# kemingy/rabitq

Measured on AMD Instinct MI355X. Metric: queries/sec at recall@10>=0.95, 100Mx128; HBM GB/s on popcount scan, higher is better.
Workload: dtype exact integer dot (fp6 MFMA, v_dot8_u32_u4) + f32

## Files before the change

### rabitq_amd/csrc/common.h

```cpp
#pragma once
#include <hip/hip_runtime.h>
#include <stdint.h>

#pragma clang fp contract(off)

#define RQ_WAVE 64

typedef float f32x2 __attribute__((ext_vector_type(2)));

__host__ __device__ __forceinline__ int32_t ord32_from_f32(float x) {
    int32_t bits = __builtin_bit_cast(int32_t, x);
    uint32_t mask = ((uint32_t)(bits >> 31)) >> 1;
    return bits ^ (int32_t)mask;
}
__host__ __device__ __forceinline__ float ord32_to_f32(int32_t key) {
    uint32_t mask = ((uint32_t)(key >> 31)) >> 1;
    return __builtin_bit_cast(float, key ^ (int32_t)mask);
}
__host__ __device__ __forceinline__ uint32_t ord32_biased(float x) {
    return (uint32_t)ord32_from_f32(x) ^ 0x80000000u;
}
__host__ __device__ __forceinline__ float ord32_unbias(uint32_t u) {
    return ord32_to_f32((int32_t)(u ^ 0x80000000u));
}

__device__ __forceinline__ float reduce8_lanes(float acc) {
    acc = acc + __shfl_xor(acc, 4, 8);
    acc = acc + __shfl_xor(acc, 1, 8);
    acc = acc + __shfl_xor(acc, 2, 8);
    return acc;
}
__device__ __forceinline__ float reduce8_regs(const float (&a)[8]) {
    float c0 = a[0] + a[4], c1 = a[1] + a[5], c2 = a[2] + a[6], c3 = a[3] + a[7];
    return (c0 + c1) + (c2 + c3);
}

__device__ __forceinline__ int32_t cvtps_epi32(float x) {
    if (x >= -2147483648.0f && x < 2147483648.0f) return (int32_t)rintf(x);
    return (int32_t)0x80000000;
}

struct __attribute__((aligned(16))) SurvRec {
    uint32_t pos;
    uint32_t slot;
    float rough;
    float accurate;
};
__device__ __forceinline__ uint64_t surv_key(const SurvRec &r) {
    return ((uint64_t)r.slot << 32) | r.pos;
}

struct __attribute__((aligned(16))) RunRec {
    uint32_t pos;
    uint32_t slot;
// ... 192 lines not shown
```

### rabitq_amd/csrc/host_plan.h

```cpp
#pragma once
struct QueryParams {
    uint32_t nq, len, probe, topk;
    bool heuristic;
    uint32_t cap, hcap;
    const float *thr_init = nullptr;
    bool seg_final = false;
    bool ext_lists = false;
    const rq_filter *filter = nullptr;
    bool range = false;
};

struct QueryIO {
    const float *d_q = nullptr;
    float *out_dist = nullptr;
    uint32_t *out_id = nullptr, *out_n = nullptr;
    const uint32_t *ext_cluster = nullptr;
    const float *ext_dist = nullptr;
    const float *thr_init = nullptr;
};
struct QueryCall {
    rq_index *idx = nullptr;
    const rq_filter *filter = nullptr;
    uint32_t len = 0, probe = 0, topk = 0;
    bool heuristic = false;
// ... 23 lines not shown
#define RQ_MAX_PROBE 16384u
#define RQ_SB_FILT_REACH 65536u

#define RQ_PREP_SHAPES(X) X(128, 16, 2, 16, 2) X(64, 16, 1, 16, 4) X(256, 32, 2, 8, 2) X(512, 32, 4, 8, 1) X(768, 32, 6, 8, 1) X(1024, 32, 8, 8, 1)

struct StagePlan {
    uint32_t s_lo, s_hi;
    uint64_t span, est_pairs;
    bool matrix;
    bool cluster_major;
    bool ranked;
    bool additive;
    bool arena_stage;
    bool placed;
    bool want_table;
    uint32_t slot_hi, stage_pairs;
    uint32_t dense_cells;
    uint32_t tile, tiles_per_group;
};

struct PassPlan {
    uint32_t nprobe, npairs;
    uint32_t dbg;
    bool large;
    bool small;
    uint32_t sb_nstages, sb_lo[RQ_SB_MAX_STAGES], sb_hi[RQ_SB_MAX_STAGES], sb_final_lo;
    bool sb_whole, sb_fill_final;
    bool will_list;
    bool placed;
    bool fin_additive;
// ... 10 lines not shown
    const uint64_t total_max = std::min<uint64_t>((uint64_t)nprobe * idx->max_list_len, idx->n);
    uint64_t lo = 0, hi = first_hi;
    const uint64_t avg = std::max<uint64_t>(1, idx->n / std::max<uint32_t>(idx->nonempty_lists, 1));
    uint64_t settle = std::min(settle_cap, std::max<uint64_t>(avg, std::min<uint64_t>(idx->max_list_len, 16 * avg)));
    if (pl.large) settle = std::max<uint64_t>(1, settle * settle_pct / 100);
    while (lo < total_max) {
        const bool last = hi >= total_max || lo >= settle || pl.nstages + 1 == RQ_MAX_STAGES;
        pl.st[pl.nstages++] = StagePlan{(uint32_t)lo, last ? 0xFFFFFFFFu : (uint32_t)hi};
        if (last) break;
        lo = hi;
        hi = std::min<uint64_t>(hi * growth, 0xFFFFFFF0ull);
        if (lo < 2 * avg && 2 * hi > 2 * avg) hi = 2 * avg;
        if (lo < settle && hi > settle) hi = settle;
    }
}

static void plan_pass(const rq_index *idx, const QueryParams &qp, bool has_row_map, bool ext_lists, PassPlan &pl) {
    const uint32_t dim = idx->dim, k = idx->k, W = idx->W;
    const uint32_t nq = qp.nq, nprobe = std::min(qp.probe, k), topk = qp.topk;
    const uint32_t npairs = nq * nprobe;
    const rq_filter *filt = qp.filter;
    const bool large = rq_large_batch(nq), fused = scan_is_fused(W);
    pl = PassPlan{};
    pl.nprobe = nprobe, pl.npairs = npairs, pl.large = large;
    const uint32_t min_len = filt ? 0u : idx->min_list_len;
    const int impl = g_scan_impl.load();
    pl.dbg = (uint32_t)g_scan_dbg.load();
    const int gate_opt = g_scan_gate.load(), rank_opt = g_group_rank.load(), tt_opt = g_scan_tile_table.load(), gopt = g_stage_growth.load();
    const bool dense_opt = g_dense_dir.load() != 0, additive_loose = idx->additive_loose.load() != 0;
    const uint64_t settle_pct = (uint64_t)g_stage_settle_pct.load();
// ... 48 lines not shown
                     (gate_opt == 2 || !additive_loose);
        s.slot_hi = nprobe;
        if (s.cluster_major && min_len > 0 && !ext_lists && s.s_hi != 0xFFFFFFFFu)
            s.slot_hi = (uint32_t)std::min<uint64_t>(nprobe, (uint64_t)(s.s_hi - 1) / min_len + 1);
        s.stage_pairs = nq * s.slot_hi;
        s.ranked = s.cluster_major && k <= 32768 &&
                   (rank_opt == 2 || (rank_opt == 1 && s.stage_pairs >= 16 * RQ_RANK_ITEMS && s.stage_pairs / RQ_RANK_ITEMS >= k / 256));
        s.tile = s.matrix ? scan_mfma_tile(W, s.arena_stage, s.additive) : scan_tile(W);
        s.tiles_per_group = ceil_div(std::min<uint64_t>(idx->max_list_len, s.s_hi), s.tile);
        const uint64_t grid_blocks = (uint64_t)k * s.tiles_per_group, real_tiles = idx->n / s.tile + k;
        s.want_table = s.cluster_major && fused && s.s_hi >= idx->max_list_len && (tt_opt == 2 || (tt_opt == 1 && grid_blocks > 4 * real_tiles));
        if (large && !s.matrix && fused && dense_opt && s.s_hi != 0xFFFFFFFFu && !(qp.seg_final && s.span > qp.cap)) {
            const uint64_t cells = (uint64_t)((s.s_hi - 1) >> 6) - (s.s_lo >> 6) + 2ull * s.slot_hi + 2;
            if (cells <= qp.cap) s.dense_cells = (uint32_t)cells;
        }
    }

#define RQ_X(D, LP, R, PPB, PP) \
    if (dim == D) pl.prep_lp = LP, pl.prep_r = R, pl.prep_ppb = PPB, pl.prep_pp = PP;
    RQ_PREP_SHAPES(RQ_X)
#undef RQ_X
    const bool prep_dim = pl.prep_lp != 0;
    pl.will_list = !pl.small && (filt || (idx->nonempty_lists * 2 < k && npairs >= 65536)) && g_pair_split.load() != 0 && prep_dim;
    if (g_prep_placement.load() != 0 && !pl.small && !filt && !ext_lists && !has_row_map && !qp.thr_init && !qp.seg_final && !pl.will_list &&
        prep_dim && fused && pl.nstages) {
        StagePlan &fin = pl.st[pl.nstages - 1];
        pl.placed = fin.s_hi == 0xFFFFFFFFu && fin.matrix && fin.ranked;
        for (uint32_t i = 0; i + 1 < pl.nstages; ++i) pl.placed = pl.placed && !pl.st[i].matrix;
        fin.placed = pl.placed;
        pl.fin_additive = pl.placed && fin.additive;
// ... 13 lines not shown

    if (pl.dbg & 16384) {
        fprintf(stderr, "[rabitq_hip] plan: pass nq=%u nprobe=%u large=%d small=%d will_list=%d placed=%d fin_additive=%d qn_slots=%u nstages=%u seg_final=%d sb_nstages=%u sb_whole=%d\n",
                nq, nprobe, (int)pl.large, (int)pl.small, (int)pl.will_list, (int)pl.placed, (int)pl.fin_additive, pl.qn_slots, pl.nstages, (int)qp.seg_final,
                pl.small ? pl.sb_nstages : 0u, (int)(pl.small && pl.sb_whole));
        for (uint32_t i = 0; pl.small && i < pl.sb_nstages; ++i)
            fprintf(stderr, "[rabitq_hip] plan: sb_stage=%u lo=%u hi=%u\n", i, pl.sb_lo[i], pl.sb_hi[i]);
        for (uint32_t i = 0; i < pl.nstages; ++i) {
            const StagePlan &s = pl.st[i];
            fprintf(stderr, "[rabitq_hip] stage %u: [%u, %u) span %llu est_pairs %llu %s\n", i, s.s_lo, s.s_hi, (unsigned long long)s.span,
                    (unsigned long long)s.est_pairs, s.matrix ? "matrix cores" : (s.cluster_major ? "VALU, list-major" : "VALU, pair-major"));
            if (s.placed) fprintf(stderr, "[rabitq_hip] stage %u: placed ahead of the quantisation (%s gate)\n", i, pl.fin_additive ? "additive" : "bf16");
            fprintf(stderr, "[rabitq_hip] plan: stage=%u lo=%u hi=%u matrix=%d cluster_major=%d ranked=%d additive=%d arena=%d placed=%d table=%d dense_cells=%u slot_hi=%u\n",
                    i, s.s_lo, s.s_hi, (int)s.matrix, (int)s.cluster_major, (int)s.ranked, (int)s.additive, (int)s.arena_stage, (int)s.placed, (int)s.want_table,
                    s.dense_cells, s.slot_hi);
        }
    }
}
```

### rabitq_amd/csrc/host_query.h

```cpp
#pragma once
static rq_status ws_prepare(const rq_index *idx, Workspace &ws, const QueryParams &qp) {
    const uint32_t nprobe = std::min(qp.probe, idx->k);
    const uint64_t nq = qp.nq, npairs = nq * nprobe;
    RQC(ws_ensure_stream(ws));
    RQC(ws.qpad.ensure(nq * idx->dim));
    RQC(ws.y.ensure(nq * idx->dim));
    if (!qp.ext_lists) RQC(ws.dist.ensure(nq * idx->k));
    RQC(ws.probe_dist.ensure(npairs));
    RQC(ws.probe_cluster.ensure(npairs));
    RQC(ws.scal.ensure(npairs));
    if (!scan_is_fused(idx->W)) RQC(ws.planes.ensure(npairs * 4 * idx->W));
    RQC(ws.qnib.ensure(npairs * 8 * idx->W));
    RQC(ws.qf6.ensure(npairs * 12 * idx->W));
    RQC(ws.rough_cnt.ensure(nq));
    RQC(ws.totals.ensure(16));
    RQC(ws.stat.ensure(256));
    RQC(ws.recs.ensure((npairs + 32ull * idx->k + 32) * (12ull * idx->W + 2 + RQ_REC_TAIL)));
    RQC(ws.grp_cnt.ensure(idx->k + 4));
    RQC(ws.grp_start.ensure(idx->k + 1));
    RQC(ws.q_hist.ensure(idx->k + 2));
    RQC(ws.q_start.ensure(idx->k + 2));
    RQC(ws.q_order.ensure(nq));
    RQC(ws.thr.ensure(nq));
    RQC(ws.surv.ensure(nq * qp.cap));
// ... 496 lines not shown
                flags |= 2u;
            }
            auto finish = topk < 64 ? sb_finish_kernel<true> : sb_finish_kernel<false>;
            finish<<<nq, fin_threads, (size_t)dim * sizeof(float) + (2 * RQ_SBF_RUNS + RQ_SBF_RECS) * 16, st>>>(
                ws.surv.p, ws.runs.p, ws.surv_cnt.p, seg, idx->view(), qpad, dim, topk, rs, probe_cluster, nprobe, flags,
                idx->map_ids.p, io.out_dist, io.out_id, io.out_n, ws.rough_cnt.p, ws.totals.p);
            sb_results_done = true;
        } else {
            auto finish = qp.heuristic ? stage_finish_kernel<true> : stage_finish_kernel<false>;
            finish<<<nq, fin_threads, (size_t)dim * sizeof(float), st>>>(ws.surv.p, ws.runs.p, ws.surv_cnt.p, seg, idx->view(), qpad, dim, topk, rs,
                                                                         probe_cluster, nprobe, flags);
        }
        pf.end();
    }

    void stage_finish_large(StageRun &r) {
        const uint32_t dense_cells = r.s.dense_cells;
        const QSeg &seg = r.seg;
        pf.begin(PF_RERANK);
        const uint32_t gx = std::max(1u, std::min(16u, 4096u / std::max(nq, 1u)));
        const bool prefilter = (r.no > 0 || qp.thr_init) && !(pl.dbg & 512);
        if (idx->base_q8.p && prefilter)
            accurate_filtered8_kernel<<<dim3(gx, nq), 256, (size_t)dim * sizeof(float) + (nprobe <= RQ_ACC8_LDS_PROBES ? (size_t)nprobe * 16 : 0), st>>>(
                ws.surv.p, ws.surv_cnt.p, seg, idx->base.p, idx->base_q8.p, idx->list_q8.p, qpad, dim, rerank_order, ws.thr.p,
                probe_cluster, nprobe, ws.nshadow.p, k);
        else if (idx->base_h.p && prefilter)
            accurate_filtered_kernel<<<dim3(gx, nq), 256, (size_t)dim * sizeof(float), st>>>(
                ws.surv.p, ws.surv_cnt.p, seg, idx->base.p, idx->base_h.p, qpad, dim, rerank_order, ws.thr.p,
                ws.nshadow.p);
        else if (idx->split_rows && prefilter)
            accurate_split_kernel<<<dim3(gx, nq), 256, (size_t)dim * sizeof(float) + (nprobe <= RQ_ACC8_LDS_PROBES ? (size_t)nprobe * 16 : 0), st>>>(
                ws.surv.p, ws.surv_cnt.p, seg, idx->view(), qpad, dim, rerank_order, ws.thr.p, probe_cluster, nprobe, ws.nshadow.p);
        else
            accurate_kernel<<<dim3(gx, nq), 256, (size_t)dim * sizeof(float), st>>>(ws.surv.p, ws.surv_cnt.p, seg, idx->view(), qpad, dim,
                                                                                    rerank_order, probe_cluster, nprobe);
        if (qp.range)
            range_count_kernel<<<ceil_div(nq, 4), 256, 0, st>>>(ws.surv.p, ws.surv_cnt.p, qp.cap, ws.thr.p, nq, ws.range_hits.p, ws.need.p,
// ... 68 lines not shown
    const size_t total_span = pf.spans.size() ? pf.spans.size() - 1 : 0;
    if (pl.small) {
        RQC(c.small_front());
    } else {
        RQC(c.rotate_coarse());
        if (pl.placed) RQC(c.place_final());
        pf.begin(PF_PREP);
        RQC(c.quantise());
        RQC(c.orders_state());
        pf.end();
    }
    for (uint32_t i = 0; i < pl.nstages; ++i) {
        StageRun r{pl.st[i], i};
        RQC(c.stage_group_fill(r));
        RQC(c.stage_scan(r));
        if (!qp.range && !pl.large && qp.cap <= 4 * RQ_DEFAULT_CAP) c.stage_finish_small(r);
        else c.stage_finish_large(r);
    }
    RQC(c.results(total_span));
    if (defer) return RQ_OK;
    return finish_pass(idx, ws, res, prof_acc);
}
```

### rabitq_amd/csrc/host_state.h

```cpp
#pragma once
static thread_local std::string g_err;
static rq_status fail(rq_status s, const std::string &msg) {
    g_err = msg;
    return s;
}
#define HIPC(expr)                                                                                   \
    do {                                                                                             \
        hipError_t _e = (expr);                                                                      \
        if (_e != hipSuccess)                                                                        \
            return fail(_e == hipErrorOutOfMemory ? RQ_ERR_OOM : RQ_ERR_HIP,                         \
                        std::string(#expr) + ": " + hipGetErrorString(_e));                          \
    } while (0)
#define RQC(expr)                        \
    do {                                 \
        rq_status _s = (expr);           \
        if (_s != RQ_OK) return _s;      \
    } while (0)

static rq_status ensure_device() {
    int count = 0;
    hipError_t e = hipGetDeviceCount(&count);
    if (e != hipSuccess || count == 0)
        return fail(RQ_ERR_NO_DEVICE, "no HIP device visible (librabitq_hip has no CPU fallback)");
    return RQ_OK;
// ... 699 lines not shown
    static hipError_t err = hipSuccess;
    static const char *what = "";
    std::call_once(once, [] {
        auto set = [&](const void *fn, int bytes, const char *name) {
            if (err != hipSuccess) return;
            err = hipFuncSetAttribute(fn, hipFuncAttributeMaxDynamicSharedMemorySize, bytes);
            if (err != hipSuccess) what = name;
        };
        set(reinterpret_cast<const void *>(select_probe_kernel), 140 * 1024, "select_probe_kernel");
        set(reinterpret_cast<const void *>(coarse_dist_kernel<4>), 140 * 1024, "coarse_dist_kernel<4>");
        set(reinterpret_cast<const void *>(coarse_dist_kernel<8>), 140 * 1024, "coarse_dist_kernel<8>");
        set(reinterpret_cast<const void *>(assign_generic_kernel<8>), 140 * 1024, "assign_generic_kernel<8>");
        set(reinterpret_cast<const void *>(merge_smallest_u64_kernel), 16384 * 8, "merge_smallest_u64_kernel");
        set(reinterpret_cast<const void *>(group_rank_kernel), 32768 * 4, "group_rank_kernel");
        set(reinterpret_cast<const void *>(sb_front_kernel), 140 * 1024, "sb_front_kernel");
        set(reinterpret_cast<const void *>(sort_runs_mid_kernel), RQ_SORT_MID_LDS_WORDS * 8, "sort_runs_mid_kernel");
        set(reinterpret_cast<const void *>(range_sort_block_kernel<1024, RQ_RANGE_TILE>), RQ_RANGE_TILE * 8, "range_sort_block_kernel");
        set(reinterpret_cast<const void *>(range_sort_tile_kernel), RQ_RANGE_TILE * 8, "range_sort_tile_kernel");
        set(reinterpret_cast<const void *>(assign_approx_kernel<6, 1>), (int)assign_lds_bytes<6, 1>(), "assign_approx_kernel<6,1>");
        set(reinterpret_cast<const void *>(assign_approx_kernel<8, 1>), (int)assign_lds_bytes<8, 1>(), "assign_approx_kernel<8,1>");
        set(reinterpret_cast<const void *>(assign_approx_kernel<12, 1>), (int)assign_lds_bytes<12, 1>(), "assign_approx_kernel<12,1>");
        set(reinterpret_cast<const void *>(coarse_approx_kernel<6, 1>), (int)assign_lds_bytes<6, 1>(), "coarse_approx_kernel<6,1>");
        set(reinterpret_cast<const void *>(coarse_approx_kernel<8, 1>), (int)assign_lds_bytes<8, 1>(), "coarse_approx_kernel<8,1>");
        set(reinterpret_cast<const void *>(coarse_approx_kernel<12, 1>), (int)assign_lds_bytes<12, 1>(), "coarse_approx_kernel<12,1>");
        set(reinterpret_cast<const void *>(sb_finish_kernel<true>), 104 * 1024, "sb_finish_kernel");
        set(reinterpret_cast<const void *>(sb_finish_kernel<false>), 104 * 1024, "sb_finish_kernel");
#define RQ_SBQ_ATTR(WW)                                                                                  \
    set(reinterpret_cast<const void *>(sb_query_kernel<WW, 0, false>), 120 * 1024, "sb_query_kernel");   \
    set(reinterpret_cast<const void *>(sb_query_kernel<WW, 1, false>), 120 * 1024, "sb_query_kernel");   \
    set(reinterpret_cast<const void *>(sb_query_kernel<WW, 2, false>), 120 * 1024, "sb_query_kernel")
// ... 26 lines not shown
```

### rabitq_amd/csrc/kernels_rerank.h

```cpp
#pragma once
#include "common.h"

__global__ __launch_bounds__(256) void accurate_flat_kernel(const uint32_t *__restrict__ pos, uint32_t m,
                                                            const BaseView base,
                                                            const float *__restrict__ q, uint32_t dim,
                                                            float *__restrict__ out) {
    const uint32_t l = threadIdx.x & 7;
    uint32_t i = blockIdx.x * 32 + (threadIdx.x >> 3);
    if (i >= m) return;
    const RowRef x = base.row(pos[i], dim);
    float acc = 0.0f;
    for (uint32_t c = 0; c < dim; c += 8) {
        float d = rq_row_get(x, dim, c + l) - q[c + l];
        acc = fmaf(d, d, acc);
    }
    acc = reduce8_lanes(acc);
    if (l == 0) out[i] = acc;
}

__device__ __forceinline__ void exact_l2_acc64(const float4 (&xv)[8], const float *q, float &a0, float &a1, float &a2, float &a3) {
#pragma unroll
    for (int u = 0; u < 8; ++u) {
        const float4 qv = *reinterpret_cast<const float4 *>(q + 8 * u);
        const float d0 = xv[u].x - qv.x, d1 = xv[u].y - qv.y, d2 = xv[u].z - qv.z, d3 = xv[u].w - qv.w;
// ... 74 lines not shown
template <class P>
__device__ __forceinline__ void rerank_prefiltered(P &pol, SurvRec *__restrict__ surv, const unsigned long long *__restrict__ surv_cnt,
                                                   const QSeg &seg, const float *__restrict__ qpad, uint32_t dim,
                                                   const uint32_t *__restrict__ order, const float *__restrict__ thr_start,
                                                   uint32_t *__restrict__ nshadow) {
    constexpr int V = P::V;
    extern __shared__ __attribute__((aligned(16))) float acc_q[];
    __shared__ uint32_t queue[256 * V];
    __shared__ uint32_t qn;
    const uint32_t b = order ? order[blockIdx.y] : blockIdx.y;
    const uint32_t n = (uint32_t)surv_cnt[b];
    if (n > seg.capof(b) || n == 0) return;
    SurvRec *recs = surv + seg.at(b);
    const uint32_t hf = threadIdx.x & 1, pair = threadIdx.x >> 1;
    const uint32_t i_first = blockIdx.x * (128 * V), stride = gridDim.x * (128 * V);
    SurvRec nxt[V];
#pragma unroll
    for (int v = 0; v < V; ++v) nxt[v] = recs[i_first + 128 * v + pair < n ? i_first + 128 * v + pair : 0u];
    for (uint32_t c = threadIdx.x * 4; c < dim; c += 1024)
        *reinterpret_cast<float4 *>(acc_q + c) = *reinterpret_cast<const float4 *>(qpad + (uint64_t)b * dim + c);
    pol.stage(acc_q + dim, b);
    if (threadIdx.x == 0) qn = 0;
    __syncthreads();
    const float thr = thr_start ? thr_start[b] : __builtin_inff();
    const bool test = thr > 1e-30f && thr < 3.0e38f;
    const float eps = (float)(dim / 4 + 64) * 5.9604645e-8f, down = 1.0f - eps, up = 1.0f + eps;
    auto exact_of = [&](uint32_t j) {
        const float r = pol.exact(recs[j], acc_q, hf);
        if (hf == 0) recs[j].accurate = r;
    };
    uint32_t rejected = 0;
    for (uint32_t i0 = i_first; i0 < n; i0 += stride) {
        uint32_t iv[V];
        bool exact[V];
        SurvRec cur[V];
#pragma unroll
        for (int v = 0; v < V; ++v) {
            iv[v] = i0 + 128 * v + pair, exact[v] = iv[v] < n, cur[v] = nxt[v];
            nxt[v] = recs[iv[v] + stride < n ? iv[v] + stride : 0u];
        }
        if (test && exact[0]) {
            float dt[V], err[V];
            pol.bound(cur, acc_q, hf, up, dt, err);
#pragma unroll
            for (int v = 0; v < V; ++v) {
                const float t = sqrtf(dt[v] * down) * down - err[v] * up;
                if (exact[v] && t > 0.0f && (t * t) * (down * down) > thr) {
                    exact[v] = false;
                    if (hf == 0) recs[iv[v]].accurate = __builtin_inff();
                    ++rejected;
                }
            }
        }
#pragma unroll
        for (int v = 0; v < V; ++v)
            if (exact[v] && hf == 0) queue[atomicAdd(&qn, 1u)] = iv[v];
        __syncthreads();
        uint32_t waiting = qn;
        __syncthreads();
        if (waiting >= 128) {
            do {
                exact_of(queue[waiting - 128 + pair]);
                waiting -= 128;
            } while (V > 1 && waiting >= 128);
            if (threadIdx.x == 0) qn = waiting;
            __syncthreads();
        }
    }
    if (pair < qn) exact_of(queue[pair]);
    uint32_t rj = hf == 0 ? rejected : 0u;
#pragma unroll
    for (int o = 32; o >= 1; o >>= 1) rj += __shfl_xor(rj, o, 64);
    if ((threadIdx.x & 63) == 0 && rj) atomicAdd(&nshadow[b], rj);
}

template <class Widen>
__device__ __forceinline__ void shadow16_bound(const uint16_t *__restrict__ x, const float *q_lds, uint32_t dim, uint32_t hf, Widen widen,
                                               float &dt, float &nx) {
    float d0 = 0.0f, d1 = 0.0f, n0 = 0.0f, n1 = 0.0f;
    for (uint32_t c = 0; c < dim; c += 128) {
        uint4 xv[8];
        const bool full = dim - c >= 128;
// ... 8 lines not shown
            float xe[8];
            widen(xv[u], xe);
            const float e0 = xe[0] - qa.x, e1 = xe[1] - qa.y, e2 = xe[2] - qa.z, e3 = xe[3] - qa.w;
            const float e4 = xe[4] - qb.x, e5 = xe[5] - qb.y, e6 = xe[6] - qb.z, e7 = xe[7] - qb.w;
            d0 = fmaf(e0, e0, d0), d1 = fmaf(e1, e1, d1), d0 = fmaf(e2, e2, d0), d1 = fmaf(e3, e3, d1);
            d0 = fmaf(e4, e4, d0), d1 = fmaf(e5, e5, d1), d0 = fmaf(e6, e6, d0), d1 = fmaf(e7, e7, d1);
            n0 = fmaf(xe[0], xe[0], n0), n1 = fmaf(xe[1], xe[1], n1), n0 = fmaf(xe[2], xe[2], n0), n1 = fmaf(xe[3], xe[3], n1);
            n0 = fmaf(xe[4], xe[4], n0), n1 = fmaf(xe[5], xe[5], n1), n0 = fmaf(xe[6], xe[6], n0), n1 = fmaf(xe[7], xe[7], n1);
        }
    }
    dt = d0 + d1, nx = n0 + n1;
    dt += __shfl_xor(dt, 1, 2), nx += __shfl_xor(nx, 1, 2);
}

struct ShadowHalf {
    static constexpr int V = 1;
    const float *base;
    const _Float16 *base_h;
    uint32_t dim;
    __device__ __forceinline__ void stage(float *, uint32_t) const {}
    __device__ __forceinline__ void bound(const SurvRec (&cur)[1], const float *q_lds, uint32_t hf, float up, float (&dt)[1], float (&err)[1]) const {
        float nx;
        shadow16_bound(reinterpret_cast<const uint16_t *>(base_h + (uint64_t)cur[0].pos * dim) + 8 * hf, q_lds, dim, hf,
                       [](const uint4 w, float (&xe)[8]) {
                           const rq_half8 h = __builtin_bit_cast(rq_half8, w);
#pragma unroll
                           for (int e = 0; e < 8; ++e) xe[e] = (float)h[e];
                       },
                       dt[0], nx);
        const float abs_err = sqrtf((float)dim) * 3.0e-8f;
// ... 7 lines not shown
    }
};
__global__ __launch_bounds__(256) void accurate_filtered_kernel(SurvRec *__restrict__ surv,
                                                                const unsigned long long *__restrict__ surv_cnt,
                                                                const QSeg seg, const float *__restrict__ base,
                                                                const _Float16 *__restrict__ base_h,
                                                                const float *__restrict__ qpad, uint32_t dim,
                                                                const uint32_t *__restrict__ order,
                                                                const float *__restrict__ thr_start,
                                                                uint32_t *__restrict__ nshadow) {
    ShadowHalf pol{base, base_h, dim};
    rerank_prefiltered(pol, surv, surv_cnt, seg, qpad, dim, order, thr_start, nshadow);
}

struct ShadowPlane {
    static constexpr int V = 1;
    const BaseView &base;
    const uint32_t *probe_row;
    uint32_t nprobe, dim;
    const ListTier *ltl;
    __device__ __forceinline__ void stage(float *behind, uint32_t b) {
        probe_row += (uint64_t)b * nprobe;
        if (base.host == nullptr || nprobe > RQ_ACC8_LDS_PROBES) return;
        ListTier *l = reinterpret_cast<ListTier *>(behind);
        for (uint32_t sl = threadIdx.x; sl < nprobe; sl += 256)
            l[sl] = probe_row[sl] < base.k ? base.lt[probe_row[sl]] : ListTier{0u, 0u, 0u, 0u};
        ltl = l;
    }
    __device__ __forceinline__ RowRef row_of(const SurvRec &r) const {
        if (!base.host) return RowRef{base.dev + (uint64_t)r.pos * dim, base.split != 0};
// ... 107 lines not shown
#pragma unroll
    for (int o = 32; o >= 1; o >>= 1) {
        const float a = __shfl_xor(emax, o, 64), b = __shfl_xor(nmax, o, 64);
        emax = a > emax ? a : emax, nmax = b > nmax ? b : nmax;
    }
    if ((threadIdx.x & 63) == 0) smax[threadIdx.x >> 6] = emax, snorm[threadIdx.x >> 6] = nmax;
    __syncthreads();
    if (threadIdx.x == 0) {
        for (int w2 = 1; w2 < 4; ++w2) emax = smax[w2] > emax ? smax[w2] : emax, nmax = snorm[w2] > nmax ? snorm[w2] : nmax;
        atomicMax(reinterpret_cast<unsigned int *>(&list_q8[c].z), __builtin_bit_cast(unsigned int, emax));
        const float nrm = sqrtf(nmax) * (1.0f + (float)(dim + 8) * 6.0e-8f);
        if (row_norms) atomicMax(reinterpret_cast<unsigned int *>(&list_q8[c].w), __builtin_bit_cast(unsigned int, nrm));
    }
}

struct ShadowQ8 {
    static constexpr int V = 2;
    const float *base;
    const uint8_t *base_q8;
    const float4 *list_q8;
    const uint32_t *probe_row;
    uint32_t nprobe, nlists, dim;
    const float4 *lpar;
    __device__ __forceinline__ void stage(float *behind, uint32_t b) {
        probe_row += (uint64_t)b * nprobe;
        if (nprobe > RQ_ACC8_LDS_PROBES) return;
        float4 *l = reinterpret_cast<float4 *>(behind);
        for (uint32_t sl = threadIdx.x; sl < nprobe; sl += 256)
            l[sl] = probe_row[sl] < nlists ? list_q8[probe_row[sl]] : make_float4(0.0f, 1.0f, __builtin_inff(), __builtin_inff());
        lpar = l;
    }
    __device__ __forceinline__ void bound(const SurvRec (&cur)[2], const float *q_lds, uint32_t hf, float up, float (&dt)[2], float (&err)[2]) const {
        const uint32_t ngrp = dim / 16;
        float4 par[2];
        const uint8_t *x[2];
#pragma unroll
        for (int v = 0; v < 2; ++v) {
            par[v] = lpar ? lpar[cur[v].slot] : list_q8[probe_row[cur[v].slot]];
            x[v] = base_q8 + (uint64_t)cur[v].pos * dim;
        }
        float d0[2] = {0.0f, 0.0f}, d1[2] = {0.0f, 0.0f};
        for (uint32_t g0 = hf; g0 < ngrp; g0 += 8) {
            uint4 cv[2][4];
#pragma unroll
            for (int v = 0; v < 2; ++v)
#pragma unroll
                for (int u = 0; u < 4; ++u)
                    if (g0 + 2 * u < ngrp) cv[v][u] = *reinterpret_cast<const uint4 *>(x[v] + 16 * (g0 + 2 * u));
#pragma unroll
            for (int u = 0; u < 4; ++u) {
                if (!(g0 + 2 * u < ngrp)) continue;
                const float *q = q_lds + 16 * (g0 + 2 * u);
#pragma unroll
                for (int wi = 0; wi < 4; ++wi) {
                    const float4 qa = *reinterpret_cast<const float4 *>(q + 4 * wi);
#pragma unroll
                    for (int v = 0; v < 2; ++v) {
                        const uint32_t wv = wi == 0 ? cv[v][u].x : (wi == 1 ? cv[v][u].y : (wi == 2 ? cv[v][u].z : cv[v][u].w));
                        const float e0 = fmaf(par[v].y, (float)(wv & 255u), par[v].x) - qa.x;
                        const float e1 = fmaf(par[v].y, (float)((wv >> 8) & 255u), par[v].x) - qa.y;
                        const float e2 = fmaf(par[v].y, (float)((wv >> 16) & 255u), par[v].x) - qa.z;
                        const float e3 = fmaf(par[v].y, (float)(wv >> 24), par[v].x) - qa.w;
                        d0[v] = fmaf(e0, e0, d0[v]), d1[v] = fmaf(e1, e1, d1[v]), d0[v] = fmaf(e2, e2, d0[v]), d1[v] = fmaf(e3, e3, d1[v]);
                    }
                }
                asm volatile("" ::: "memory");
            }
        }
        const float sqd = sqrtf((float)dim) * 1.001f;
#pragma unroll
        for (int v = 0; v < 2; ++v) {
            dt[v] = d0[v] + d1[v];
            dt[v] += __shfl_xor(dt[v], 1, 2);
            err[v] = q8_row_norms(dim) ? par[v].w * up : (par[v].z * up) * sqd;
        }
    }
    __device__ __forceinline__ float exact(const SurvRec &r, const float *q_lds, uint32_t hf) const {
        return exact_l2_pair(base + (uint64_t)r.pos * dim + 4 * hf, q_lds, dim, hf);
    }
};
#ifndef RQ_ACC8_WAVES
#define RQ_ACC8_WAVES 4
#endif
__global__ __launch_bounds__(256, RQ_ACC8_WAVES) void accurate_filtered8_kernel(SurvRec *__restrict__ surv,
                                                                 const unsigned long long *__restrict__ surv_cnt,
                                                                 const QSeg seg, const float *__restrict__ base,
                                                                 const uint8_t *__restrict__ base_q8, const float4 *__restrict__ list_q8,
                                                                 const float *__restrict__ qpad, uint32_t dim,
                                                                 const uint32_t *__restrict__ order,
                                                                 const float *__restrict__ thr_start,
                                                                 const uint32_t *__restrict__ probe_cluster, uint32_t nprobe,
                                                                 uint32_t *__restrict__ nshadow, uint32_t nlists) {
    ShadowQ8 pol{base, base_q8, list_q8, probe_cluster, nprobe, nlists, dim, nullptr};
    rerank_prefiltered(pol, surv, surv_cnt, seg, qpad, dim, order, thr_start, nshadow);
}

__global__ __launch_bounds__(256) void accurate_kernel(SurvRec *__restrict__ surv,
                                                       const unsigned long long *__restrict__ surv_cnt,
                                                       const QSeg seg, const BaseView base,
                                                       const float *__restrict__ qpad, uint32_t dim,
                                                       const uint32_t *__restrict__ order,
                                                       const uint32_t *__restrict__ probe_cluster, uint32_t nprobe) {
    extern __shared__ __attribute__((aligned(16))) float acc_q[];
    const uint32_t b = order ? order[blockIdx.y] : blockIdx.y;
    const uint32_t n = (uint32_t)surv_cnt[b];
    if (n > seg.capof(b) || n == 0) return;
    for (uint32_t c = threadIdx.x * 4; c < dim; c += 1024)
        *reinterpret_cast<float4 *>(acc_q + c) = *reinterpret_cast<const float4 *>(qpad + (uint64_t)b * dim + c);
    __syncthreads();
    accurate_rows(surv + seg.at(b), n, base, acc_q, dim, blockIdx.x * 128 + (threadIdx.x >> 1), gridDim.x * 128,
                  probe_cluster + (uint64_t)b * nprobe);
// ... 3 lines not shown
```

### rabitq_amd/csrc/kernels_scan_mfma.h

```cpp
#pragma once
#include "kernels_scan_common.h"

typedef int v8i32 __attribute__((ext_vector_type(8)));
typedef __bf16 bf16x8 __attribute__((ext_vector_type(8)));
typedef __bf16 bf16x2 __attribute__((ext_vector_type(2)));
typedef int v16i32 __attribute__((ext_vector_type(16)));
__device__ __forceinline__ int imax3(int a, int b, int c) {
    const int m = a > b ? a : b;
    return m > c ? m : c;
}
typedef int v4i32 __attribute__((ext_vector_type(4)));
#ifndef RQ_F32X16_DEFINED
#define RQ_F32X16_DEFINED
typedef float f32x16 __attribute__((ext_vector_type(16)));
#endif

__device__ __forceinline__ void glds16(const void *gsrc, uint32_t lds_dst) {
    uint32_t keep;
    asm volatile("s_mov_b32 %0, m0\n\ts_mov_b32 m0, %2\n\ts_nop 0\n\tglobal_load_lds_dwordx4 %1, off\n\ts_mov_b32 m0, %0"
                 : "=&s"(keep)
                 : "v"(gsrc), "s"(lds_dst)
                 : "memory");
}
__device__ __forceinline__ uint32_t lds_addr(const void *p) {
    return (uint32_t)(uintptr_t)(const __attribute__((address_space(3))) void *)p;
}

template <int W, int NT, bool ARENA, bool ADD, bool FILT>
__global__ __launch_bounds__((64 * scan_mfma_waves<W, ARENA>()), scan_mfma_blocks_per_cu<W>() ) void scan_mfma_kernel(const uint32_t *__restrict__ codes,
                                                           const float4 *__restrict__ factors,
                                                           const uint32_t *__restrict__ offsets,
                                                           const uint32_t *__restrict__ grp_start,
                                                           const uint32_t *__restrict__ grp_cnt,
                                                           const uint32_t *__restrict__ recs,
                                                           SurvRec *__restrict__ surv, RunRec *__restrict__ runs,
                                                           unsigned long long *__restrict__ surv_cnt,
                                                           unsigned long long *__restrict__ stat ,
                                                           const uint4 *__restrict__ tile_table,
                                                           const float4 *__restrict__ list_uref ,
                                                           const float4 *__restrict__ grp_vref ,
                                                           const ScanArgs a) {
// ... 520 lines not shown
```

### rabitq_amd/csrc/rabitq_hip.hip

```cpp
#include "../../include/rabitq_hip.h"

#include <hip/hip_runtime.h>

#include <algorithm>
#include <charconv>
#include <chrono>
#include <atomic>
#include <cmath>
#include <cstdio>
#include <cstdlib>
#include <cstring>
#include <memory>
#include <mutex>
#include <random>
#include <string>
#include <thread>
#include <vector>
#include <sys/stat.h>
#include <dlfcn.h>
#include <queue>
#include <map>

#include "common.h"
#include "kernels_build.h"
// ... 980 lines not shown
    }
    if (std::string(name) == "rerank_shadow") {
        if (value < 0 || value > 2) return fail(RQ_ERR_INVALID, "rerank_shadow must be 0 (never), 1 (fp16 rows when they fit) or 2 (8-bit rows when they fit)");
        g_rerank_shadow = value;
        return RQ_OK;
    }
    if (std::string(name) == "scan_gate") {
        if (value < 0 || value > 2) return fail(RQ_ERR_INVALID, "scan_gate must be 0, 1 or 2");
        g_scan_gate = value;
        return RQ_OK;
    }
    if (std::string(name) == "scan_debug") {
#ifdef RQ_DEV_ABLATIONS
        const int allowed = 0x7FFFFFFF;
#else
        const int allowed = 128 | 512 | 2048 | 4096 | 16384;
#endif
        if (value < 0 || (value & ~allowed)) return fail(RQ_ERR_INVALID, "scan_debug: this bit exists in the developer build only (librabitq_hip_dev.so)");
        g_scan_dbg = value;
        return RQ_OK;
    }
    return fail(RQ_ERR_INVALID, std::string("unknown option ") + name);
}

rq_status rq_set_profiling(int level) {
    if (level < 0 || level > 2) return fail(RQ_ERR_INVALID, "profiling level must be 0, 1 or 2");
    g_profiling = level;
    return RQ_OK;
}
rq_status rq_last_profile(rq_profile_t *out) {
    if (!out) return fail(RQ_ERR_INVALID, "null argument");
// ... 181 lines not shown
```

Baseline: 3.896 million.

## Stream 8-bit rerank rows into an LDS double-buffered ring via async global-to-LDS loads

Adds a rerank kernel specialization for dims 64/128/192/256 that prefetches the next batch of 8-bit shadow rows straight into a per-wave LDS ring with global_load_lds, double-buffered and with a swizzled layout. The rows for iteration i+1 load while the bound for iteration i is computed, which hides the latency of the scattered row gathers. The q8 bound computation is factored into a shared helper, and a second record lookahead (nxt2) is added. In exchange the kernel uses a lot of LDS and fewer waves per CU, and the hand-rolled vmcnt waits are fragile.

```diff
diff --git a/rabitq_amd/csrc/common.h b/rabitq_amd/csrc/common.h
--- a/rabitq_amd/csrc/common.h
+++ b/rabitq_amd/csrc/common.h
@@ -38,6 +38,17 @@
 __device__ __forceinline__ int32_t cvtps_epi32(float x) {
     if (x >= -2147483648.0f && x < 2147483648.0f) return (int32_t)rintf(x);
     return (int32_t)0x80000000;
+}
+
+__device__ __forceinline__ void glds16(const void *gsrc, uint32_t lds_dst) {
+    uint32_t keep;
+    asm volatile("s_mov_b32 %0, m0\n\ts_mov_b32 m0, %2\n\ts_nop 0\n\tglobal_load_lds_dwordx4 %1, off\n\ts_mov_b32 m0, %0"
+                 : "=&s"(keep)
+                 : "v"(gsrc), "s"(lds_dst)
+                 : "memory");
+}
+__device__ __forceinline__ uint32_t lds_addr(const void *p) {
+    return (uint32_t)(uintptr_t)(const __attribute__((address_space(3))) void *)p;
 }
 
 struct __attribute__((aligned(16))) SurvRec {
diff --git a/rabitq_amd/csrc/host_plan.h b/rabitq_amd/csrc/host_plan.h
--- a/rabitq_amd/csrc/host_plan.h
+++ b/rabitq_amd/csrc/host_plan.h
@@ -61,6 +61,9 @@
     bool arena_stage;
     bool placed;
     bool want_table;
+    bool prefilter;
+    bool rerank_q8;
+    bool rerank_ring;
     uint32_t slot_hi, stage_pairs;
     uint32_t dense_cells;
     uint32_t tile, tiles_per_group;
@@ -101,6 +104,12 @@
         if (lo < settle && hi > settle) hi = settle;
     }
 }
+
+static inline uint32_t rerank_ring_lds(uint32_t dim, uint32_t nprobe) { return dim * 4u + nprobe * 16u + q8_ring_bytes(RQ_RING_V, dim); }
+static inline bool rerank_ring_rule(uint32_t dim, uint32_t nprobe, uint32_t dbg) {
+    return !(dbg & 32768u) && (dim == 64 || dim == 128 || dim == 192 || dim == 256) && nprobe <= RQ_ACC8_LDS_PROBES;
+}
+static inline bool finish_large(const PassPlan &pl, const QueryParams &qp) { return qp.range || pl.large || qp.cap > 4 * RQ_DEFAULT_CAP; }
 
 static void plan_pass(const rq_index *idx, const QueryParams &qp, bool has_row_map, bool ext_lists, PassPlan &pl) {
     const uint32_t dim = idx->dim, k = idx->k, W = idx->W;
@@ -179,6 +188,9 @@
             const uint64_t cells = (uint64_t)((s.s_hi - 1) >> 6) - (s.s_lo >> 6) + 2ull * s.slot_hi + 2;
             if (cells <= qp.cap) s.dense_cells = (uint32_t)cells;
         }
+        s.prefilter = (i > 0 || qp.thr_init) && !(pl.dbg & 512);
+        s.rerank_q8 = s.prefilter && idx->base_q8.p != nullptr;
+        s.rerank_ring = s.rerank_q8 && rerank_ring_rule(dim, nprobe, pl.dbg);
     }
 
 #define RQ_X(D, LP, R, PPB, PP) \
@@ -222,6 +234,7 @@
             fprintf(stderr, "[rabitq_hip] plan: stage=%u lo=%u hi=%u matrix=%d cluster_major=%d ranked=%d additive=%d arena=%d placed=%d table=%d dense_cells=%u slot_hi=%u\n",
                     i, s.s_lo, s.s_hi, (int)s.matrix, (int)s.cluster_major, (int)s.ranked, (int)s.additive, (int)s.arena_stage, (int)s.placed, (int)s.want_table,
                     s.dense_cells, s.slot_hi);
+            if (s.rerank_q8 && finish_large(pl, qp)) fprintf(stderr, "[rabitq_hip] stage %u: rerank=%s\n", i, s.rerank_ring ? "ring" : "regs");
         }
     }
 }
diff --git a/rabitq_amd/csrc/host_query.h b/rabitq_amd/csrc/host_query.h
--- a/rabitq_amd/csrc/host_query.h
+++ b/rabitq_amd/csrc/host_query.h
@@ -534,13 +534,25 @@
         pf.end();
     }
 
+    template <int NPC>
+    void launch_ring8(uint32_t gx, const QSeg &seg) {
+        accurate_ring8_kernel<RQ_RING_V, NPC><<<dim3(gx, nq), 256, rerank_ring_lds(dim, nprobe), st>>>(
+            ws.surv.p, ws.surv_cnt.p, seg, idx->base.p, idx->base_q8.p, idx->list_q8.p, qpad, rerank_order, ws.thr.p, probe_cluster, nprobe,
+            ws.nshadow.p, k);
+    }
+
     void stage_finish_large(StageRun &r) {
         const uint32_t dense_cells = r.s.dense_cells;
         const QSeg &seg = r.seg;
         pf.begin(PF_RERANK);
         const uint32_t gx = std::max(1u, std::min(16u, 4096u / std::max(nq, 1u)));
-        const bool prefilter = (r.no > 0 || qp.thr_init) && !(pl.dbg & 512);
-        if (idx->base_q8.p && prefilter)
+        const bool prefilter = r.s.prefilter;
+        if (r.s.rerank_ring) {
+            if (dim == 64) launch_ring8<4>(gx, seg);
+            else if (dim == 128) launch_ring8<8>(gx, seg);
+            else if (dim == 192) launch_ring8<12>(gx, seg);
+            else launch_ring8<16>(gx, seg);
+        } else if (r.s.rerank_q8)
             accurate_filtered8_kernel<<<dim3(gx, nq), 256, (size_t)dim * sizeof(float) + (nprobe <= RQ_ACC8_LDS_PROBES ? (size_t)nprobe * 16 : 0), st>>>(
                 ws.surv.p, ws.surv_cnt.p, seg, idx->base.p, idx->base_q8.p, idx->list_q8.p, qpad, dim, rerank_order, ws.thr.p,
                 probe_cluster, nprobe, ws.nshadow.p, k);
@@ -639,8 +651,8 @@
         StageRun r{pl.st[i], i};
         RQC(c.stage_group_fill(r));
         RQC(c.stage_scan(r));
-        if (!qp.range && !pl.large && qp.cap <= 4 * RQ_DEFAULT_CAP) c.stage_finish_small(r);
-        else c.stage_finish_large(r);
+        if (finish_large(pl, qp)) c.stage_finish_large(r);
+        else c.stage_finish_small(r);
     }
     RQC(c.results(total_span));
     if (defer) return RQ_OK;
diff --git a/rabitq_amd/csrc/host_state.h b/rabitq_amd/csrc/host_state.h
--- a/rabitq_amd/csrc/host_state.h
+++ b/rabitq_amd/csrc/host_state.h
@@ -737,6 +737,10 @@
         set(reinterpret_cast<const void *>(merge_smallest_u64_kernel), 16384 * 8, "merge_smallest_u64_kernel");
         set(reinterpret_cast<const void *>(group_rank_kernel), 32768 * 4, "group_rank_kernel");
         set(reinterpret_cast<const void *>(sb_front_kernel), 140 * 1024, "sb_front_kernel");
+        set(reinterpret_cast<const void *>(accurate_ring8_kernel<RQ_RING_V, 4>), 156 * 1024, "accurate_ring8_kernel<4>");
+        set(reinterpret_cast<const void *>(accurate_ring8_kernel<RQ_RING_V, 8>), 156 * 1024, "accurate_ring8_kernel<8>");
+        set(reinterpret_cast<const void *>(accurate_ring8_kernel<RQ_RING_V, 12>), 156 * 1024, "accurate_ring8_kernel<12>");
+        set(reinterpret_cast<const void *>(accurate_ring8_kernel<RQ_RING_V, 16>), 156 * 1024, "accurate_ring8_kernel<16>");
         set(reinterpret_cast<const void *>(sort_runs_mid_kernel), RQ_SORT_MID_LDS_WORDS * 8, "sort_runs_mid_kernel");
         set(reinterpret_cast<const void *>(range_sort_block_kernel<1024, RQ_RANGE_TILE>), RQ_RANGE_TILE * 8, "range_sort_block_kernel");
         set(reinterpret_cast<const void *>(range_sort_tile_kernel), RQ_RANGE_TILE * 8, "range_sort_tile_kernel");
diff --git a/rabitq_amd/csrc/kernels_rerank.h b/rabitq_amd/csrc/kernels_rerank.h
--- a/rabitq_amd/csrc/kernels_rerank.h
+++ b/rabitq_amd/csrc/kernels_rerank.h
@@ -112,9 +112,13 @@
     SurvRec *recs = surv + seg.at(b);
     const uint32_t hf = threadIdx.x & 1, pair = threadIdx.x >> 1;
     const uint32_t i_first = blockIdx.x * (128 * V), stride = gridDim.x * (128 * V);
-    SurvRec nxt[V];
+    SurvRec nxt[V], nxt2[V];
 #pragma unroll
     for (int v = 0; v < V; ++v) nxt[v] = recs[i_first + 128 * v + pair < n ? i_first + 128 * v + pair : 0u];
+    if constexpr (P::RING) {
+#pragma unroll
+        for (int v = 0; v < V; ++v) nxt2[v] = recs[i_first + stride + 128 * v + pair < n ? i_first + stride + 128 * v + pair : 0u];
+    }
     for (uint32_t c = threadIdx.x * 4; c < dim; c += 1024)
         *reinterpret_cast<float4 *>(acc_q + c) = *reinterpret_cast<const float4 *>(qpad + (uint64_t)b * dim + c);
     pol.stage(acc_q + dim, b);
@@ -128,14 +132,33 @@
         if (hf == 0) recs[j].accurate = r;
     };
     uint32_t rejected = 0;
+    if constexpr (P::RING) {
+        pol.ring_slot = 0;
+        if (test && i_first < n) pol.ring_issue(nxt, 0u);
+    }
     for (uint32_t i0 = i_first; i0 < n; i0 += stride) {
         uint32_t iv[V];
         bool exact[V];
         SurvRec cur[V];
-#pragma unroll
-        for (int v = 0; v < V; ++v) {
-            iv[v] = i0 + 128 * v + pair, exact[v] = iv[v] < n, cur[v] = nxt[v];
-            nxt[v] = recs[iv[v] + stride < n ? iv[v] + stride : 0u];
+        if constexpr (P::RING) {
+#pragma unroll
+            for (int v = 0; v < V; ++v) {
+                iv[v] = i0 + 128 * v + pair, exact[v] = iv[v] < n, cur[v] = nxt[v], nxt[v] = nxt2[v];
+                asm volatile("" ::"v"(nxt[v].pos), "v"(nxt[v].slot));
+            }
+            if (test) {
+                const bool more = i0 + stride < n;
+                if (more) pol.ring_issue(nxt, pol.ring_slot ^ 1u);
+                pol.ring_wait(more);
+            }
+#pragma unroll
+            for (int v = 0; v < V; ++v) nxt2[v] = recs[iv[v] + 2 * stride < n ? iv[v] + 2 * stride : 0u];
+        } else {
+#pragma unroll
+            for (int v = 0; v < V; ++v) {
+                iv[v] = i0 + 128 * v + pair, exact[v] = iv[v] < n, cur[v] = nxt[v];
+                nxt[v] = recs[iv[v] + stride < n ? iv[v] + stride : 0u];
+            }
         }
         if (test && exact[0]) {
             float dt[V], err[V];
@@ -164,6 +187,7 @@
             if (threadIdx.x == 0) qn = waiting;
             __syncthreads();
         }
+        if constexpr (P::RING) pol.ring_slot ^= 1u;
     }
     if (pair < qn) exact_of(queue[pair]);
     uint32_t rj = hf == 0 ? rejected : 0u;
@@ -202,6 +226,7 @@
 }
 
 struct ShadowHalf {
+    static constexpr bool RING = false;
     static constexpr int V = 1;
     const float *base;
     const _Float16 *base_h;
@@ -239,6 +264,7 @@
 }
 
 struct ShadowPlane {
+    static constexpr bool RING = false;
     static constexpr int V = 1;
     const BaseView &base;
     const uint32_t *probe_row;
@@ -376,8 +402,52 @@
     }
 }
 
+template <int V, class Piece>
+__device__ __forceinline__ void q8_bound(const float4 (&par)[V], Piece piece, const float *q_lds, uint32_t dim, uint32_t hf, float up,
+                                         float (&dt)[V], float (&err)[V]) {
+    const uint32_t ngrp = dim / 16;
+    float d0[V], d1[V];
+#pragma unroll
+    for (int v = 0; v < V; ++v) d0[v] = 0.0f, d1[v] = 0.0f;
+    for (uint32_t g0 = hf; g0 < ngrp; g0 += 8) {
+        uint4 cv[V][4];
+#pragma unroll
+        for (int v = 0; v < V; ++v)
+#pragma unroll
+            for (int u = 0; u < 4; ++u)
+                if (g0 + 2 * u < ngrp) cv[v][u] = piece(v, g0 + 2 * u);
+#pragma unroll
+        for (int u = 0; u < 4; ++u) {
+            if (!(g0 + 2 * u < ngrp)) continue;
+            const float *q = q_lds + 16 * (g0 + 2 * u);
+#pragma unroll
+            for (int wi = 0; wi < 4; ++wi) {
+                const float4 qa = *reinterpret_cast<const float4 *>(q + 4 * wi);
+#pragma unroll
+                for (int v = 0; v < V; ++v) {
+                    const uint32_t wv = wi == 0 ? cv[v][u].x : (wi == 1 ? cv[v][u].y : (wi == 2 ? cv[v][u].z : cv[v][u].w));
+                    const float e0 = fmaf(par[v].y, (float)(wv & 255u), par[v].x) - qa.x;
+                    const float e1 = fmaf(par[v].y, (float)((wv >> 8) & 255u), par[v].x) - qa.y;
+                    const float e2 = fmaf(par[v].y, (float)((wv >> 16) & 255u), par[v].x) - qa.z;
+                    const float e3 = fmaf(par[v].y, (float)(wv >> 24), par[v].x) - qa.w;
+                    d0[v] = fmaf(e0, e0, d0[v]), d1[v] = fmaf(e1, e1, d1[v]), d0[v] = fmaf(e2, e2, d0[v]), d1[v] = fmaf(e3, e3, d1[v]);
+                }
+            }
+            asm volatile("" ::: "memory");
+        }
+    }
+    const float sqd = sqrtf((float)dim) * 1.001f;
+#pragma unroll
+    for (int v = 0; v < V; ++v) {
+        dt[v] = d0[v] + d1[v];
+        dt[v] += __shfl_xor(dt[v], 1, 2);
+        err[v] = q8_row_norms(dim) ? par[v].w * up : (par[v].z * up) * sqd;
+    }
+}
+
 struct ShadowQ8 {
     static constexpr int V = 2;
+    static constexpr bool RING = false;
     const float *base;
     const uint8_t *base_q8;
     const float4 *list_q8;
@@ -393,7 +463,6 @@
         lpar = l;
     }
     __device__ __forceinline__ void bound(const SurvRec (&cur)[2], const float *q_lds, uint32_t hf, float up, float (&dt)[2], float (&err)[2]) const {
-        const uint32_t ngrp = dim / 16;
         float4 par[2];
         const uint8_t *x[2];
 #pragma unroll
@@ -401,41 +470,7 @@
             par[v] = lpar ? lpar[cur[v].slot] : list_q8[probe_row[cur[v].slot]];
             x[v] = base_q8 + (uint64_t)cur[v].pos * dim;
         }
-        float d0[2] = {0.0f, 0.0f}, d1[2] = {0.0f, 0.0f};
-        for (uint32_t g0 = hf; g0 < ngrp; g0 += 8) {
-            uint4 cv[2][4];
-#pragma unroll
-            for (int v = 0; v < 2; ++v)
-#pragma unroll
-                for (int u = 0; u < 4; ++u)
-                    if (g0 + 2 * u < ngrp) cv[v][u] = *reinterpret_cast<const uint4 *>(x[v] + 16 * (g0 + 2 * u));
-#pragma unroll
-            for (int u = 0; u < 4; ++u) {
-                if (!(g0 + 2 * u < ngrp)) continue;
-                const float *q = q_lds + 16 * (g0 + 2 * u);
-#pragma unroll
-                for (int wi = 0; wi < 4; ++wi) {
-                    const float4 qa = *reinterpret_cast<const float4 *>(q + 4 * wi);
-#pragma unroll
-                    for (int v = 0; v < 2; ++v) {
-                        const uint32_t wv = wi == 0 ? cv[v][u].x : (wi == 1 ? cv[v][u].y : (wi == 2 ? cv[v][u].z : cv[v][u].w));
-                        const float e0 = fmaf(par[v].y, (float)(wv & 255u), par[v].x) - qa.x;
-                        const float e1 = fmaf(par[v].y, (float)((wv >> 8) & 255u), par[v].x) - qa.y;
-                        const float e2 = fmaf(par[v].y, (float)((wv >> 16) & 255u), par[v].x) - qa.z;
-                        const float e3 = fmaf(par[v].y, (float)(wv >> 24), par[v].x) - qa.w;
-                        d0[v] = fmaf(e0, e0, d0[v]), d1[v] = fmaf(e1, e1, d1[v]), d0[v] = fmaf(e2, e2, d0[v]), d1[v] = fmaf(e3, e3, d1[v]);
-                    }
-                }
-                asm volatile("" ::: "memory");
-            }
-        }
-        const float sqd = sqrtf((float)dim) * 1.001f;
-#pragma unroll
-        for (int v = 0; v < 2; ++v) {
-            dt[v] = d0[v] + d1[v];
-            dt[v] += __shfl_xor(dt[v], 1, 2);
-            err[v] = q8_row_norms(dim) ? par[v].w * up : (par[v].z * up) * sqd;
-        }
+        q8_bound<2>(par, [&](int v, uint32_t g) { return *reinterpret_cast<const uint4 *>(x[v] + 16 * g); }, q_lds, dim, hf, up, dt, err);
     }
     __device__ __forceinline__ float exact(const SurvRec &r, const float *q_lds, uint32_t hf) const {
         return exact_l2_pair(base + (uint64_t)r.pos * dim + 4 * hf, q_lds, dim, hf);
@@ -457,6 +492,73 @@
     rerank_prefiltered(pol, surv, surv_cnt, seg, qpad, dim, order, thr_start, nshadow);
 }
 
+template <int NPC>
+__device__ __forceinline__ uint32_t q8_ring_piece(uint32_t r, uint32_t g) {
+    if constexpr (NPC == 4) return g ^ (2u * ((r >> 2) & 1u));
+    if constexpr (NPC == 8) return g ^ (2u * ((r >> 1) & 3u));
+    if constexpr (NPC == 16) return g ^ (2u * (r & 7u));
+    return g;
+}
+__host__ __device__ constexpr uint32_t q8_ring_bytes(uint32_t v, uint32_t dim) { return 2u * 4u * 32u * v * dim; }
+template <int VV, int NPC>
+struct ShadowQ8Ring : ShadowQ8 {
+    static constexpr int V = VV;
+    static constexpr bool RING = true;
+    static constexpr uint32_t DIM = 16u * NPC, WAVE_BYTES = 32u * VV * DIM, SLOT_BYTES = 4u * WAVE_BYTES, NI = VV * NPC / 2;
+    uint32_t rows;
+    uint32_t wave_lds;
+    uint32_t ring_slot;
+    __device__ __forceinline__ void stage(float *behind, uint32_t b) {
+        ShadowQ8::stage(behind, b);
+        const uint32_t ring = 4u * DIM + 16u * nprobe, wave = __builtin_amdgcn_readfirstlane(threadIdx.x >> 6);
+        wave_lds = lds_addr(dyn()) + ring + wave * WAVE_BYTES;
+        rows = ring + wave * WAVE_BYTES + ((threadIdx.x & 63u) >> 1) * DIM;
+    }
+    __device__ __forceinline__ static const uint8_t *dyn() {
+        extern __shared__ __attribute__((aligned(16))) uint8_t rq_ring_lds[];
+        return rq_ring_lds;
+    }
+    __device__ __forceinline__ void ring_issue(const SurvRec (&nx)[VV], uint32_t slot) const {
+        const uint32_t lane = threadIdx.x & 63u, dst = wave_lds + slot * SLOT_BYTES;
+#pragma unroll
+        for (uint32_t j = 0; j < NI; ++j) {
+            const uint32_t v = j / (NPC / 2), at = 64u * (j % (NPC / 2)) + lane, r = at / NPC, p = at % NPC;
+            const uint32_t pos = (uint32_t)__shfl((int)nx[v < VV ? v : 0].pos, (int)(2u * r), 64);
+            glds16(base_q8 + (uint64_t)pos * DIM + 16u * q8_ring_piece<NPC>(r, p), dst + 1024u * j);
+        }
+    }
+    __device__ __forceinline__ void ring_wait(bool issued) const {
+        if (issued) asm volatile("s_waitcnt vmcnt(%0)" ::"n"(NI) : "memory");
+        else asm volatile("s_waitcnt vmcnt(0)" ::: "memory");
+    }
+    __device__ __forceinline__ void bound(const SurvRec (&cur)[VV], const float *q_lds, uint32_t hf, float up, float (&dt)[VV], float (&err)[VV]) const {
+        float4 par[VV];
+#pragma unroll
+        for (int v = 0; v < VV; ++v) par[v] = reinterpret_cast<const float4 *>(dyn() + 4u * DIM)[cur[v].slot];
+        const uint8_t *x = dyn() + rows + ring_slot * SLOT_BYTES;
+        const uint32_t r = (threadIdx.x & 63u) >> 1;
+        q8_bound<VV>(par, [&](int v, uint32_t g) { return *reinterpret_cast<const uint4 *>(x + v * (32u * DIM) + 16u * q8_ring_piece<NPC>(r, g)); },
+                     q_lds, DIM, hf, up, dt, err);
+    }
+};
+#ifndef RQ_RING_V
+#define RQ_RING_V 1
+#endif
+__host__ __device__ constexpr int q8_ring_waves(int npc) { return npc <= 8 ? 4 : 2; }
+template <int VV, int NPC>
+__global__ __launch_bounds__(256, q8_ring_waves(NPC)) void accurate_ring8_kernel(SurvRec *__restrict__ surv, const unsigned long long *__restrict__ surv_cnt,
+                                                             const QSeg seg, const float *__restrict__ base,
+                                                             const uint8_t *__restrict__ base_q8, const float4 *__restrict__ list_q8,
+                                                             const float *__restrict__ qpad, const uint32_t *__restrict__ order,
+                                                             const float *__restrict__ thr_start,
+                                                             const uint32_t *__restrict__ probe_cluster, uint32_t nprobe,
+                                                             uint32_t *__restrict__ nshadow, uint32_t nlists) {
+    ShadowQ8Ring<VV, NPC> pol;
+    pol.base = base, pol.base_q8 = base_q8, pol.list_q8 = list_q8, pol.probe_row = probe_cluster, pol.nprobe = nprobe, pol.nlists = nlists;
+    pol.dim = 16u * NPC, pol.lpar = nullptr;
+    rerank_prefiltered(pol, surv, surv_cnt, seg, qpad, 16u * NPC, order, thr_start, nshadow);
+}
+
 __global__ __launch_bounds__(256) void accurate_kernel(SurvRec *__restrict__ surv,
                                                        const unsigned long long *__restrict__ surv_cnt,
                                                        const QSeg seg, const BaseView base,
diff --git a/rabitq_amd/csrc/kernels_scan_mfma.h b/rabitq_amd/csrc/kernels_scan_mfma.h
--- a/rabitq_amd/csrc/kernels_scan_mfma.h
+++ b/rabitq_amd/csrc/kernels_scan_mfma.h
@@ -15,16 +15,6 @@
 typedef float f32x16 __attribute__((ext_vector_type(16)));
 #endif
 
-__device__ __forceinline__ void glds16(const void *gsrc, uint32_t lds_dst) {
-    uint32_t keep;
-    asm volatile("s_mov_b32 %0, m0\n\ts_mov_b32 m0, %2\n\ts_nop 0\n\tglobal_load_lds_dwordx4 %1, off\n\ts_mov_b32 m0, %0"
-                 : "=&s"(keep)
-                 : "v"(gsrc), "s"(lds_dst)
-                 : "memory");
-}
-__device__ __forceinline__ uint32_t lds_addr(const void *p) {
-    return (uint32_t)(uintptr_t)(const __attribute__((address_space(3))) void *)p;
-}
 
 template <int W, int NT, bool ARENA, bool ADD, bool FILT>
 __global__ __launch_bounds__((64 * scan_mfma_waves<W, ARENA>()), scan_mfma_blocks_per_cu<W>() ) void scan_mfma_kernel(const uint32_t *__restrict__ codes,
diff --git a/rabitq_amd/csrc/rabitq_hip.hip b/rabitq_amd/csrc/rabitq_hip.hip
--- a/rabitq_amd/csrc/rabitq_hip.hip
+++ b/rabitq_amd/csrc/rabitq_hip.hip
@@ -1018,7 +1018,7 @@
 #ifdef RQ_DEV_ABLATIONS
         const int allowed = 0x7FFFFFFF;
 #else
-        const int allowed = 128 | 512 | 2048 | 4096 | 16384;
+        const int allowed = 128 | 512 | 2048 | 4096 | 16384 | 32768;
 #endif
         if (value < 0 || (value & ~allowed)) return fail(RQ_ERR_INVALID, "scan_debug: this bit exists in the developer build only (librabitq_hip_dev.so)");
         g_scan_dbg = value;
```

After: 3.982 million, median of 6. 1.02x the previous value.
